# Ritesh622/Unbiased-Quantization-Distributed-Mean-Estimation

Hardware: AMD Instinct MI355X
Metric: quantize+dequantize M-vectors/sec at d=2^20 (1/2/4/8 GPU) + NMSE vs reference (higher is better)
Workload: dtype f32

## Files before the change

unbiased-quantization-distributed-mean-estimation_amd/csrc/uq_unbiased.hip:

```cpp
#include <hip/hip_runtime.h>

#include <algorithm>
#include <cstdint>
#include <type_traits>

#include "uq_internal.h"
#include "uq_unbiased_kernels.h"

namespace {

struct WsLayout {
    size_t agg_off, incl_off, map1_off, rec_off, cnt_off, part_off, l1_off, total;
    int32_t tiles;
    template <class T>
    T* at(void* ws, size_t off) const { return (T*)((char*)ws + off); }
    uint64_t* tile_row(void* ws, size_t off, int64_t j0) const { return at<uint64_t>(ws, off) + j0 * tiles; }
};

WsLayout layout(int64_t n, int64_t d, const L1Plan& plan) {
    WsLayout w{};
    const int64_t tiles = (d + kQTile - 1) / kQTile;
    w.tiles = (int32_t)tiles;
    w.agg_off = kCtrlBytes;
    w.incl_off = up256(w.agg_off + (size_t)n * tiles * sizeof(uint64_t));
// ... 72 lines not shown
    if (rc) return rc;
    if (n == 0) return UQ_OK;
    if (!l1_out) return fail(UQ_E_INVALID, "null l1_out");
    hipStream_t st = (hipStream_t)stream;
    if (d == 0) return hip_check(hipMemsetAsync(l1_out, 0, n * sizeof(float), st), "memset l1");
    return launch_l1(x, n, d, plan, w.at<float>(ws, w.part_off), l1_out, st);
}

}

namespace {

template <bool B>
using Flag = std::integral_constant<bool, B>;

template <class F>
bool select_qc(bool q, bool c, bool cv, F&& f) {
    constexpr Flag<true> Y{};
    constexpr Flag<false> N{};
    switch ((q ? 4 : 0) | (c ? 2 : 0) | (cv ? 1 : 0)) {
        case 5: f(Y, N, Y); return true;
        case 7: f(Y, Y, Y); return true;
        case 6: f(Y, Y, N); return true;
        case 3: f(N, Y, Y); return true;
        case 2: f(N, Y, N); return true;
        default: return false;
    }
}

template <class F>
bool select_vqc(bool v, bool q, bool c, bool cv, F&& f) {
    if (v) return select_qc(q, c, cv, [&](auto Q, auto C, auto CV) { f(Flag<true>{}, Q, C, CV); });
    return select_qc(q, c, cv, [&](auto Q, auto C, auto CV) { f(Flag<false>{}, Q, C, CV); });
}

int bad_selector() { return fail(UQ_E_INVALID, "internal: bad kernel selector"); }

struct PlanIn {
    int64_t n, d, ldo, ldc;
    bool x16, out16, codes16;
    bool has_out, has_codes, nib, l1_given;
    int slots;
};
struct ChunkPlan {
    int64_t nj;
    bool seg;
    int32_t prefixed, R, nseg;
};
struct UnbiasedPlan {
    int32_t form;
    bool V, Q, C, CV, l1_given;
    int64_t chunks;
    ChunkPlan last;
    int32_t tiles;
    size_t agg_off, map0_off, map1_off, rec_off, cnt_off;
};

int chunk_plan(const PlanIn& in, const UnbiasedPlan& p, int64_t j0, ChunkPlan* c) {
    c->nj = std::min<int64_t>(kMaxGridY, in.n - j0);
    const int64_t total_tiles = c->nj * (int64_t)p.tiles;
    c->seg = p.V && in.d <= ((int64_t)1 << 29) && total_tiles >= kSegMinTiles;
    c->R = 1;
    c->nseg = 1;
    if (c->seg) {
        int slots = in.slots;
        if (slots <= 0) {
            const int rc = stream_slots(&slots);
            if (rc) return rc;
        }
        const int64_t segs = std::max<int64_t>(1, slots / c->nj);
        c->R = (int32_t)((p.tiles + segs - 1) / segs);
        c->nseg = (p.tiles + c->R - 1) / c->R;
    }
    c->prefixed = c->nj >= 4 ? 1 : 0;
    return UQ_OK;
}

int plan_unbiased(const PlanIn& in, const WsLayout& w, UnbiasedPlan* p) {
    *p = UnbiasedPlan{};
    if (!in.has_out && !in.has_codes) return fail(UQ_E_INVALID, "nothing to write: out and codes are both NULL");
    const int64_t n = in.n, d = in.d;
    p->tiles = w.tiles;
    p->agg_off = w.agg_off;
    p->map0_off = w.incl_off;
    p->map1_off = w.map1_off;
    p->rec_off = w.rec_off;
    p->cnt_off = w.cnt_off;
    p->Q = in.has_out;
    p->C = in.has_codes;
    p->l1_given = in.l1_given;
    p->V = in.x16 && (!in.has_out || in.out16) && ((d % 4 == 0 && in.ldo % 4 == 0) || n == 1);
    p->CV = !in.has_codes || (in.codes16 && d % 16 == 0 && (in.ldc % 16 == 0 || n == 1));
    p->chunks = 1;
    p->last = ChunkPlan{n, false, 0, w.tiles, 1};
    if (!in.nib && d <= kSmallL1Max && p->V && n <= 0x7FFFFFFF) {
        p->form = UQ_FORM_SMALL;
        return UQ_OK;
    }
    const bool stream_form = n >= kStreamMinClients && p->V && d <= ((int64_t)1 << 29);
    if (in.nib) {
        if (!stream_form || !in.has_out || !in.has_codes)
            return fail(UQ_E_INVALID, "internal: 4-bit codes outside the stream form");
        p->form = UQ_FORM_STREAM_NIBBLES;
        p->CV = true;
        return UQ_OK;
    }
    if (stream_form) {
        p->form = UQ_FORM_STREAM;
        return UQ_OK;
    }
    p->chunks = (n + kMaxGridY - 1) / kMaxGridY;
    const int rc = chunk_plan(in, *p, (p->chunks - 1) * kMaxGridY, &p->last);
    if (rc) return rc;
    p->form = p->last.seg ? UQ_FORM_SEGMENTS : UQ_FORM_PHASED;
    return UQ_OK;
}

bool bad_pitches(bool has_out, int64_t ldo, bool has_codes, int64_t ldc, int64_t d, bool nib) {
    return (has_out && ldo < d) || (has_codes && ldc < (nib ? d / 2 : d));
}

bool bad_nibble_shape(int64_t n, int64_t d) {
    return n < kStreamMinClients || d % kNibAlign != 0 || d > ((int64_t)1 << 29);
}
int nibble_shape_error() {
    return fail(UQ_E_INVALID, "4-bit codes need n >= 256 and d a multiple of 4096 (<= 2^29)");
}

thread_local UnbiasedPlan t_last_plan{};

int export_plan(const UnbiasedPlan& p, int64_t* out, int32_t cap) {
    if (!out || cap < 0) return fail(UQ_E_INVALID, "null plan output");
    const int64_t f[UQ_PLAN_FIELDS] = {
        p.form, p.V, p.Q, p.C, p.CV, p.l1_given, p.chunks, p.last.nj, p.last.prefixed, p.last.R, p.last.nseg,
        p.tiles, (int64_t)p.agg_off, (int64_t)p.map0_off, (int64_t)p.map1_off, (int64_t)p.rec_off, (int64_t)p.cnt_off,
        (int64_t)sizeof(TileRec), kRecPerClient, kRecClients, kRecEvents, kFoldEvents};
    for (int i = 0; i < std::min<int32_t>(cap, UQ_PLAN_FIELDS); ++i) out[i] = f[i];
    return UQ_OK;
}

int unbiased_codes_impl(const float* x, float* out, int64_t ldo, int8_t* codes, int64_t ldc, int32_t* overflow,
                        int64_t n, int64_t d, int64_t m, const float* X, float Xval, const float* l1, float* l1_out,
                        int32_t T, void* ws, size_t ws_bytes, void* stream, bool nib = false) {
    L1Plan plan;
    WsLayout w;
    int rc = check_common(x, n, d, T, ws, ws_bytes, &plan, &w);
    if (rc) return rc;
    t_last_plan = UnbiasedPlan{};
    if (m < 0) return fail(UQ_E_INVALID, "m must be >= 0");
    if (bad_pitches(out, ldo, codes, ldc, d, nib)) return fail(UQ_E_INVALID, "row pitches must be >= d");
    if (n == 0 || d == 0) return UQ_OK;
    if (!X && n != 1) return fail(UQ_E_INVALID, "null X");
    const PlanIn in{n, d, ldo, ldc, aligned16(x), aligned16(out), aligned16(codes), out != nullptr, codes != nullptr,
                    nib, l1 != nullptr, 0};
    UnbiasedPlan P;
    rc = plan_unbiased(in, w, &P);
    if (rc) return rc;
    if (codes && !overflow) return fail(UQ_E_INVALID, "codes need a kmax[n] array");
    t_last_plan = P;
    hipStream_t st = (hipStream_t)stream;
    const float* l1use = l1;
    const float fm = (float)m;
    const bool vec4 = P.V, cvec = P.CV;
    if (P.form == UQ_FORM_SMALL) {
        if (!select_qc(out, codes, cvec, [&](auto Q, auto C, auto CV) {
                hipLaunchKernelGGL((quantize_small_kernel<Q(), C(), CV()>), dim3((unsigned)n), dim3(kQBlock), 0, st, x,
                                   out, codes, overflow, d, w.tiles, fm, X, Xval, l1, l1_out, ldo, ldc);
            }))
            return bad_selector();
        return hip_check(hipGetLastError(), "quantize_small_kernel launch");
    }
    if (!l1use) {
        float* l1buf = w.at<float>(ws, w.l1_off);
        rc = launch_l1(x, n, d, plan, w.at<float>(ws, w.part_off), l1buf, st);
        if (rc) return rc;
        l1use = l1buf;
    }
    if (l1_out && l1_out != l1use) {
        rc = hip_check(hipMemcpyAsync(l1_out, l1use, n * sizeof(float), hipMemcpyDeviceToDevice, st), "copy l1");
        if (rc) return rc;
    }
    const bool stream_form = P.form == UQ_FORM_STREAM || P.form == UQ_FORM_STREAM_NIBBLES;
    if (codes && !stream_form) {
        rc = hip_check(hipMemsetAsync(overflow, 0, n * sizeof(int32_t), st), "memset kmax");
        if (rc) return rc;
    }
    if (P.form == UQ_FORM_STREAM_NIBBLES) {
        hipLaunchKernelGGL((quantize_stream_kernel<true, true, true, true>), dim3((unsigned)n), dim3(kQBlock), 0, st, x,
                           out, codes, overflow, d, w.tiles, fm, X, Xval, l1use, w.tiles, 1, nullptr, ldo, ldc);
        return hip_check(hipGetLastError(), "quantize_stream_kernel (4-bit codes) launch");
    }
    if (P.form == UQ_FORM_STREAM) {
        if (!select_qc(out, codes, cvec, [&](auto Q, auto C, auto CV) {
                hipLaunchKernelGGL((quantize_stream_kernel<Q(), C(), CV()>), dim3((unsigned)n), dim3(kQBlock), 0, st, x,
                                   out, codes, overflow, d, w.tiles, fm, X, Xval, l1use, w.tiles, 1, nullptr, ldo, ldc);
            }))
            return bad_selector();
        return hip_check(hipGetLastError(), "quantize_stream_kernel launch");
    }
    for (int64_t j0 = 0; j0 < n; j0 += kMaxGridY) {
        ChunkPlan ck;
        rc = chunk_plan(in, P, j0, &ck);
        if (rc) return rc;
        const int64_t nj = ck.nj;
        const float* xj = x + j0 * d;
        float* outj = out ? out + j0 * ldo : nullptr;
        int8_t* codesj = codes ? codes + j0 * ldc : nullptr;
        int32_t* ovj = codes ? overflow + j0 : nullptr;
        const float* Xj = X ? X + j0 : nullptr;
        const float* l1j = l1use + j0;
        uint64_t* agg = w.tile_row(ws, w.agg_off, j0);
        uint64_t* pre = w.tile_row(ws, w.incl_off, j0);
        uint64_t* map1 = w.tile_row(ws, w.map1_off, j0);
        TileRec* recs = w.at<TileRec>(ws, w.rec_off);
        uint32_t* reccnt = w.at<uint32_t>(ws, w.cnt_off);
        const bool seg = ck.seg;
        const dim3 tgrid((unsigned)w.tiles, (unsigned)nj);
        const int32_t R = ck.R, nseg = ck.nseg;
        if (seg) {
            hipLaunchKernelGGL(agg_stream_kernel, dim3((unsigned)(nj * nseg)), dim3(kQBlock), 0, st, xj, d, w.tiles, fm,
                               l1j, R, nseg, agg, reccnt);
        } else if (vec4) {
            hipLaunchKernelGGL(tile_agg_kernel<true>, tgrid, dim3(kQBlock), 0, st, xj, d, w.tiles, fm, l1j, agg, reccnt);
        } else {
            hipLaunchKernelGGL(tile_agg_kernel<false>, tgrid, dim3(kQBlock), 0, st, xj, d, w.tiles, fm, l1j, agg, reccnt);
        }
        rc = hip_check(hipGetLastError(), "tile sums launch");
        if (rc) return rc;
        const int32_t prefixed = ck.prefixed;
        if (prefixed) {
            hipLaunchKernelGGL(tile_prefix_kernel, dim3((unsigned)nj), dim3(kQBlock), 0, st, agg, w.tiles);
            rc = hip_check(hipGetLastError(), "tile_prefix_kernel launch");
            if (rc) return rc;
        }
        const auto map_and_fold = [&](auto V) {
            hipLaunchKernelGGL((tile_map_kernel<V()>), tgrid, dim3(kQBlock), 0, st, xj, d, w.tiles, fm, l1j, agg, pre, map1,
                               recs, reccnt, prefixed);
            const int e = hip_check(hipGetLastError(), "tile_map_kernel launch");
            if (e) return e;
            hipLaunchKernelGGL((exact_fold_kernel<V()>), dim3((unsigned)nj), dim3(kQBlock), 0, st, xj, d, w.tiles, fm, l1j,
                               pre, map1, agg, recs, reccnt);
            return hip_check(hipGetLastError(), "exact_fold_kernel launch");
        };
        rc = vec4 ? map_and_fold(Flag<true>{}) : map_and_fold(Flag<false>{});
        if (rc) return rc;
        pre = agg;
        if (seg) {
            if (!select_qc(out, codes, cvec, [&](auto Q, auto C, auto CV) {
                    hipLaunchKernelGGL((quantize_stream_kernel<Q(), C(), CV()>), dim3((unsigned)(nj * nseg)),
                                       dim3(kQBlock), 0, st, xj, outj, codesj, ovj, d, w.tiles, fm, Xj, Xval, l1j, R, nseg,
                                       pre, ldo, ldc);
                }))
                return bad_selector();
            rc = hip_check(hipGetLastError(), "quantize_stream_kernel (segments) launch");
            if (rc) return rc;
            continue;
        }
        if (!select_vqc(vec4, out, codes, cvec, [&](auto V, auto Q, auto C, auto CV) {
                hipLaunchKernelGGL((tile_out_kernel<V(), Q(), C(), CV()>), tgrid, dim3(kQBlock), 0, st, xj, outj, codesj,
                                   ovj, d, w.tiles, fm, Xj, Xval, l1j, pre, ldo, ldc);
            }))
            return bad_selector();
        rc = hip_check(hipGetLastError(), "tile_out_kernel launch");
        if (rc) return rc;
    }
    return UQ_OK;
}

}

extern "C" {

int uq_type_unbiased_codes_ld_f32(const float* x, float* out, int64_t ldq, int8_t* codes, int64_t ldc,
                                  int32_t* overflow, int64_t n, int64_t d, int64_t m, const float* X, const float* l1,
                                  float* l1_out, int32_t T, void* ws, size_t ws_bytes, void* stream) {
    if (n > 0 && d > 0 && !X) return fail(UQ_E_INVALID, "null X");
    return unbiased_codes_impl(x, out, ldq, codes, ldc, overflow, n, d, m, X, 0.0f, l1, l1_out, T, ws, ws_bytes,
                               stream);
}

int uq_type_unbiased_nibbles_ld_f32(const float* x, float* out, int64_t ldq, uint8_t* nib, int64_t ldn,
                                    int32_t* kmax, int64_t n, int64_t d, int64_t m, const float* X, const float* l1,
                                    float* l1_out, int32_t T, void* ws, size_t ws_bytes, void* stream) {
    if (n < 0 || d < 0) return fail(UQ_E_INVALID, "n and d must be >= 0");
    if (n == 0 || d == 0) return UQ_OK;
    if (!x || !out || !nib || !kmax || !X) return fail(UQ_E_INVALID, "null pointer (x, out, codes, kmax and X are required)");
    if (bad_nibble_shape(n, d)) return nibble_shape_error();
    if (ldq < d || ldq % 4 != 0 || ldn < d / 2 || ldn % 16 != 0 || !aligned16(x) || !aligned16(out) || !aligned16(nib))
        return fail(UQ_E_INVALID, "4-bit codes need 16-byte aligned rows: ldq >= d, ldq % 4 == 0, ldn >= d/2, ldn % 16 == 0");
    return unbiased_codes_impl(x, out, ldq, (int8_t*)nib, ldn, kmax, n, d, m, X, 0.0f, l1, l1_out, T, ws, ws_bytes,
                               stream, true);
}

int uq_nibbles_q_mean_ld_f32(const uint8_t* nib, int64_t ldn, const float* q, int64_t ldq, const float* l1,
                             const int32_t* kmax, int64_t n, int64_t d, int64_t m, float n_div, int32_t accumulate,
                             float* est, void* stream) {
    if (n < 0 || d < 0 || m < 0) return fail(UQ_E_INVALID, "n, d and m must be >= 0");
    if (d == 0) return UQ_OK;
    if (!est || (n > 0 && (!nib || !l1 || !kmax || !q))) return fail(UQ_E_INVALID, "null pointer (q is required)");
    if (d % kNibAlign != 0 || ldq < d || ldq % 4 != 0 || ldn < d / 2 || ldn % 4 != 0 || !aligned16(est) ||
        (n > 0 && (!aligned16(q) || ((uintptr_t)nib & 3u))))
        return fail(UQ_E_INVALID, "4-bit code mean: d % 4096 == 0, ldq >= d (multiple of 4), ldn >= d/2 (multiple of 4), "
                                  "16-byte aligned est and q");
    const int64_t blocks = d / (kCodesMeanThreads * kMeanCpt);
    if (blocks > 0x7FFFFFFF) return fail(UQ_E_INVALID, "d too large");
    hipLaunchKernelGGL(nibbles_mean_kernel, dim3((unsigned)blocks), dim3(kCodesMeanThreads), 0, (hipStream_t)stream, nib,
                       ldn, l1, kmax, n, d, (float)m, n_div, accumulate, est, q, ldq);
    return hip_check(hipGetLastError(), "nibbles_mean_kernel launch");
}

int uq_type_unbiased_codes_f32(const float* x, float* out, int8_t* codes, int32_t* overflow, int64_t n, int64_t d,
                               int64_t m, const float* X, const float* l1, float* l1_out, int32_t T, void* ws,
                               size_t ws_bytes, void* stream) {
    return uq_type_unbiased_codes_ld_f32(x, out, d, codes, d, overflow, n, d, m, X, l1, l1_out, T, ws, ws_bytes,
                                         stream);
}

int uq_type_unbiased_vec_f32(const float* x, float* out, int64_t d, int64_t m, float X, int32_t T, void* ws,
                             size_t ws_bytes, void* stream) {
    if (d > 0 && !out) return fail(UQ_E_INVALID, "null out");
    return unbiased_codes_impl(x, out, d, nullptr, d, nullptr, 1, d, m, nullptr, X, nullptr, nullptr, T, ws, ws_bytes,
                               stream);
}

int uq_type_unbiased_f32(const float* x, float* out, int64_t n, int64_t d, int64_t m, const float* X,
                         const float* l1, float* l1_out, int32_t T, void* ws, size_t ws_bytes,
                         void* stream) {
    if (n > 0 && d > 0 && !out) return fail(UQ_E_INVALID, "null out");
    return uq_type_unbiased_codes_f32(x, out, nullptr, nullptr, n, d, m, X, l1, l1_out, T, ws, ws_bytes, stream);
}

int uq_codes_decode_f32(const int8_t* codes, const float* l1, int64_t n, int64_t d, int64_t m, float* out,
                        void* stream) {
    if (n < 0 || d < 0 || m < 0) return fail(UQ_E_INVALID, "n, d and m must be >= 0");
    if (n == 0 || d == 0) return UQ_OK;
    if (!codes || !l1 || !out) return fail(UQ_E_INVALID, "null pointer");
    hipStream_t st = (hipStream_t)stream;
    const int64_t chunks = (d + kDecChunk - 1) / kDecChunk;
    if (chunks > 0x7FFFFFFF) return fail(UQ_E_INVALID, "d too large");
    const bool vec = aligned16(codes) && aligned16(out) && d % 16 == 0;
    dim3 grid((unsigned)chunks, (unsigned)n);
    if (vec)
        hipLaunchKernelGGL(codes_decode_kernel<true>, grid, dim3(256), 0, st, codes, l1, d, (float)m, out);
    else
        hipLaunchKernelGGL(codes_decode_kernel<false>, grid, dim3(256), 0, st, codes, l1, d, (float)m, out);
    return hip_check(hipGetLastError(), "codes_decode_kernel launch");
}

int uq_codes_q_mean_ld_f32(const int8_t* codes, int64_t ldc, const float* q, int64_t ldq, const float* l1,
                           const int32_t* kmax, int64_t n, int64_t d, int64_t m, float n_div, int32_t accumulate,
                           float* est, void* stream) {
    if (n < 0 || d < 0 || m < 0) return fail(UQ_E_INVALID, "n, d and m must be >= 0");
    if (d == 0) return UQ_OK;
    if (!est || (n > 0 && (!codes || !l1 || !kmax))) return fail(UQ_E_INVALID, "null pointer");
    if (q && ldq < d) return fail(UQ_E_INVALID, "ldq must be >= d");
    if (ldc < d) return fail(UQ_E_INVALID, "ldc must be >= d");
    hipStream_t st = (hipStream_t)stream;
    const bool vec = (n == 0 || aligned16(codes)) && aligned16(est) && d % 16 == 0 && ldc % 16 == 0;
    const int64_t blocks = (d + kCodesMeanThreads * kMeanCpt - 1) / (kCodesMeanThreads * kMeanCpt);
    if (blocks > 0x7FFFFFFF) return fail(UQ_E_INVALID, "d too large");
    const dim3 tb(kCodesMeanThreads);
    if (vec && d % (kCodesMeanThreads * kMeanCpt) == 0)
        hipLaunchKernelGGL((codes_mean_kernel<true, true>), dim3((unsigned)blocks), tb, 0, st, codes, ldc, l1, kmax, n,
                           d, (float)m, n_div, accumulate, est, q, ldq);
    else if (vec)
        hipLaunchKernelGGL(codes_mean_kernel<true>, dim3((unsigned)blocks), tb, 0, st, codes, ldc, l1, kmax, n, d,
                           (float)m, n_div, accumulate, est, q, ldq);
    else
        hipLaunchKernelGGL(codes_mean_kernel<false>, dim3((unsigned)blocks), tb, 0, st, codes, ldc, l1, kmax, n, d,
                           (float)m, n_div, accumulate, est, q, ldq);
    return hip_check(hipGetLastError(), "codes_mean_kernel launch");
}

int uq_codes_q_mean_f32(const int8_t* codes, const float* q, int64_t ldq, const float* l1, const int32_t* kmax,
                        int64_t n, int64_t d, int64_t m, float n_div, int32_t accumulate, float* est, void* stream) {
    return uq_codes_q_mean_ld_f32(codes, d, q, ldq, l1, kmax, n, d, m, n_div, accumulate, est, stream);
}

int uq_codes_mean_f32(const int8_t* codes, const float* l1, const int32_t* kmax, int64_t n, int64_t d, int64_t m,
                      float n_div, int32_t accumulate, float* est, void* stream) {
    return uq_codes_q_mean_f32(codes, nullptr, d, l1, kmax, n, d, m, n_div, accumulate, est, stream);
}

int uq_client_mean_f32(const float* q, int64_t n, int64_t d, int64_t ld, float n_div, int32_t accumulate,
                       float* est, void* stream) {
    if (n < 0 || d < 0) return fail(UQ_E_INVALID, "n and d must be >= 0");
    if (ld < d) return fail(UQ_E_INVALID, "ld must be >= d");
    if (d == 0) return UQ_OK;
    if (!est || (n > 0 && !q)) return fail(UQ_E_INVALID, "null pointer");
    hipStream_t st = (hipStream_t)stream;
    const bool vec4 = (n == 0 || aligned16(q)) && aligned16(est) && (d % 4 == 0) && (ld % 4 == 0);
    const int64_t threads = (d + 3) / 4;
    dim3 grid((unsigned)((threads + kMeanThreads - 1) / kMeanThreads));
    if (vec4)
        hipLaunchKernelGGL(client_mean_kernel<true>, grid, dim3(kMeanThreads), 0, st, q, n, d, ld, n_div, accumulate, est);
    else
        hipLaunchKernelGGL(client_mean_kernel<false>, grid, dim3(kMeanThreads), 0, st, q, n, d, ld, n_div, accumulate, est);
    return hip_check(hipGetLastError(), "client_mean_kernel launch");
}

int uq_type_unbiased_mean_f32(const float* x, float* out, int64_t n, int64_t d, int64_t m, const float* X,
                              const float* l1, int32_t T, float n_div, int32_t accumulate, float* est,
                              void* ws, size_t ws_bytes, void* stream) {
    if (!out) return fail(UQ_E_INVALID, "out must be non-NULL in this version");
    int rc = uq_type_unbiased_f32(x, out, n, d, m, X, l1, nullptr, T, ws, ws_bytes, stream);
    if (rc) return rc;
    return uq_client_mean_f32(out, n, d, d, n_div, accumulate, est, stream);
}

int uq_test_unbiased_plan(int64_t n, int64_t d, int64_t ldq, int64_t ldc, int32_t x_aligned, int32_t out_aligned,
                          int32_t codes_aligned, int32_t has_out, int32_t has_codes, int32_t nib, int32_t l1_given,
                          int32_t slots, int64_t* plan_out, int32_t cap) {
    L1Plan l1plan;
    if (n < 0 || d < 0) return fail(UQ_E_INVALID, "n and d must be >= 0");
    if (n > (int64_t)1 << 31 || d > (int64_t)1 << 40) return fail(UQ_E_INVALID, "n or d too large");
    if (slots < 0) return fail(UQ_E_INVALID, "slots must be >= 0");
    if (!make_plan(d, 1, &l1plan)) return fail(UQ_E_INVALID, "cannot build L1 plan");
    const WsLayout w = layout(n, d, l1plan);
    if ((int64_t)w.tiles * n > 0xFFFFFFFFll) return fail(UQ_E_INVALID, "batch too large for one call");
    if (bad_pitches(has_out, ldq, has_codes, ldc, d, nib)) return fail(UQ_E_INVALID, "row pitches must be >= d");
    UnbiasedPlan P{};
    if (n > 0 && d > 0) {
        if (nib && bad_nibble_shape(n, d)) return nibble_shape_error();
        const PlanIn in{n, d, ldq, ldc, x_aligned != 0, out_aligned != 0, codes_aligned != 0, has_out != 0,
                        has_codes != 0, nib != 0, l1_given != 0, slots};
        const int rc = plan_unbiased(in, w, &P);
        if (rc) return rc;
    }
    return export_plan(P, plan_out, cap);
}

int uq_test_last_unbiased_plan(int64_t* plan_out, int32_t cap) { return export_plan(t_last_plan, plan_out, cap); }

}
```

unbiased-quantization-distributed-mean-estimation_amd/csrc/uq_unbiased_kernels.h:

```cpp

#ifndef UQ_UNBIASED_KERNELS_H
#define UQ_UNBIASED_KERNELS_H

#include "uq_common.h"

namespace {

constexpr int kQItems = 16;
constexpr int kQTile = kQBlock * kQItems;
constexpr int64_t kStreamMinClients = 256;
constexpr int64_t kSegMinTiles = 1024;

struct AbsOp {
    static constexpr bool kHist = false;
    float den, fm;
    uint32_t *h, *zn;
    __device__ static AbsOp make(const float*, float, int64_t) { return AbsOp{0.f, 0.f, nullptr, nullptr}; }
    __device__ float operator()(float v) const { return fabsf(v); }
    __device__ void apply4(const float (&v)[4], float (&a)[4]) const {
#pragma unroll
        for (int c = 0; c < 4; ++c) a[c] += fabsf(v[c]);
    }
};

// ... 1015 lines not shown
            if (tid == 0) {
                const TileRec* lr = reinterpret_cast<const TileRec*>(s_x);
                double S = P;
                for (uint32_t e = 0; e < lr->count; ++e) {
                    const EvEntry& ev = lr->ev[e];
                    S = S + ev.run;
                    if (ev.tie) {
                        S = S + (lowbit(S) ? ev.t1 : ev.t0);
                    } else {
                        for (int k = 0; k < kQItems; ++k) S = S + (double)ev.fr[k];
                    }
                }
                sl.misc[0] = S + lr->last_run;
            }
            __syncthreads();
            P = sl.misc[0];
            __syncthreads();
        } else {
            TileRegs r;
            load_tile<VEC4>(r, x, d, tiles, (uint32_t)idx, tid);
            stage_tile<VEC4>(r, s_x, tid);
            __syncthreads();
            const int64_t t0 = (int64_t)tile * kQTile;
            const int len = (int)((d - t0) < kQTile ? (d - t0) : kQTile);
            const Binade B = binade_of(P);
            TileState st;
            TileVals tv;
            if (len == kQTile)
                tile_pass1<true, true>(s_x, tv, sl, tid, len, dp, fm, B, st);
            else
                tile_pass1<false, true>(s_x, tv, sl, tid, len, dp, fm, B, st);
            double pnext;
            (void)resolve_exact(P, B, st, tv, s_x, sl, tid, pnext);
            __syncthreads();
            P = pnext;
        }
        Pb = (uint64_t)__double_as_longlong(P);
        ++tile;
    }
}

template <bool VEC4, bool WQ, bool WC, bool CVEC>
__global__ void __launch_bounds__(kQBlock)
tile_out_kernel(const float* __restrict__ x, float* __restrict__ out, int8_t* __restrict__ codes,
                int32_t* __restrict__ overflow, int64_t d, int32_t tiles, float fm, const float* __restrict__ Xs,
                float Xval, const float* __restrict__ l1, const uint64_t* __restrict__ pre, int64_t ldo, int64_t ldc) {
    __shared__ __attribute__((aligned(16))) float s_x[kQTile];
    __shared__ float s_tab[kTab];
    __shared__ ScanLds sl;
    const int tid = threadIdx.x;
    const int32_t tile = blockIdx.x;
    const int64_t vec = blockIdx.y;
    TileRegs r;
    load_tile<VEC4>(r, x, d, tiles, (uint32_t)(vec * tiles + tile), tid);
    const float L = l1[vec];
    build_table(s_tab, tid, L, fm);
    stage_tile<VEC4>(r, s_x, tid);
    __syncthreads();
    const int64_t t0 = (int64_t)tile * kQTile;
    const int len = (int)((d - t0) < kQTile ? (d - t0) : kQTile);
    const DivPlan dp = div_plan(L);
    const double P = __longlong_as_double((long long)pre[vec * tiles + tile]);
    const Binade B = binade_of(P);
    TileState st;
    TileVals tv;
    if (len == kQTile)
        tile_pass1<true, true>(s_x, tv, sl, tid, len, dp, fm, B, st);
    else
        tile_pass1<false, true>(s_x, tv, sl, tid, len, dp, fm, B, st);
    double pnext;
    const double base = resolve_exact(P, B, st, tv, s_x, sl, tid, pnext);
    uint32_t cw[4];
    float kmax = 0.0f;
    tile_pass2<WQ, WC>(s_x, tv, s_tab, tid, base, L, fm, Xs ? Xs[vec] : Xval, cw, kmax);
    if (WC) {
        store_codes<CVEC>(codes + vec * ldc + t0, cw, len, tid);
        publish_kmax(kmax, L, overflow, vec, tid);
    }
    __syncthreads();
    if (WQ) store_tile<VEC4>(s_x, out + vec * ldo + t0, len, tid);
}

constexpr int kMeanThreads = 1024;
template <bool VEC4>
__global__ void __launch_bounds__(kMeanThreads)
client_mean_kernel(const float* __restrict__ q, int64_t n, int64_t d, int64_t ld, float n_div, int accumulate,
                   float* __restrict__ est) {
    const int64_t col = ((int64_t)blockIdx.x * blockDim.x + threadIdx.x) * 4;
    if (col >= d) return;
    if (VEC4) {
        float4 e = accumulate ? *reinterpret_cast<const float4*>(est + col) : make_float4(0.f, 0.f, 0.f, 0.f);
        int64_t j = 0;
        for (; j + 8 <= n; j += 8) {
            float4 t[8];
#pragma unroll
            for (int u = 0; u < 8; ++u) t[u] = ld_stream(reinterpret_cast<const float4*>(q + (j + u) * ld + col));
#pragma unroll
            for (int u = 0; u < 8; ++u) {
                e.x += t[u].x / n_div; e.y += t[u].y / n_div;
                e.z += t[u].z / n_div; e.w += t[u].w / n_div;
            }
        }
        for (; j < n; ++j) {
            const float4 t = *reinterpret_cast<const float4*>(q + j * ld + col);
            e.x += t.x / n_div; e.y += t.y / n_div; e.z += t.z / n_div; e.w += t.w / n_div;
        }
        *reinterpret_cast<float4*>(est + col) = e;
    } else {
        const int cnt = (int)((d - col) < 4 ? (d - col) : 4);
        for (int k = 0; k < cnt; ++k) {
            float e = accumulate ? est[col + k] : 0.f;
            for (int64_t j = 0; j < n; ++j) e += q[j * ld + col + k] / n_div;
            est[col + k] = e;
        }
    }
}

constexpr int kDecChunk = 4096;
constexpr int kMeanClients = 32;

__device__ __forceinline__ float decode_one(int8_t c, const float* tab) {
    const int ci = (int)c;
    const int k = ci ^ (ci >> 31);
    return __uint_as_float(__float_as_uint(tab[k]) ^ ((uint32_t)ci & 0x80000000u));
}

template <bool VEC>
__global__ void __launch_bounds__(256)
codes_decode_kernel(const int8_t* __restrict__ codes, const float* __restrict__ l1, int64_t d, float fm,
                    float* __restrict__ out) {
    __shared__ float tab[128];
    const int64_t vec = blockIdx.y;
    const int tid = threadIdx.x;
    const float L = l1[vec];
    if (tid < 128) tab[tid] = (L * (float)tid) / fm;
    __syncthreads();
    const int64_t i0 = (int64_t)blockIdx.x * kDecChunk + (int64_t)tid * 16;
    const int8_t* cr = codes + vec * d;
    float* orow = out + vec * d;
    if (VEC && i0 + 16 <= d) {
        const uint4 w = *reinterpret_cast<const uint4*>(cr + i0);
        const uint32_t ws[4] = {w.x, w.y, w.z, w.w};
#pragma unroll
        for (int k4 = 0; k4 < 4; ++k4) {
            float o[4];
#pragma unroll
            for (int c = 0; c < 4; ++c) o[c] = decode_one((int8_t)((ws[k4] >> (8 * c)) & 0xFF), tab);
            *reinterpret_cast<float4*>(orow + i0 + 4 * k4) = make_float4(o[0], o[1], o[2], o[3]);
        }
    } else {
        for (int64_t i = i0; i < i0 + 16 && i < d; ++i) orow[i] = decode_one(cr[i], tab);
    }
}

constexpr int kMeanCpt = 8;
constexpr int kCodesMeanThreads = 512;
constexpr int kMeanUnroll = 16;
static_assert(kMeanClients == 2 * kMeanUnroll, "two code batches per table group");

__device__ __forceinline__ void mean_load_batch(uint2 (&w)[kMeanUnroll], const int8_t* cp, int64_t ldc) {
#pragma unroll
    for (int u = 0; u < kMeanUnroll; ++u) {
        const u32x2v t = __builtin_nontemporal_load(reinterpret_cast<const u32x2v*>(cp + (int64_t)u * ldc));
        w[u] = make_uint2(t.x, t.y);
    }
}

__device__ __forceinline__ void mean_add_batch(float (&e)[kMeanCpt], const uint2 (&w)[kMeanUnroll],
                                               const float (*tabn)[256], int jj) {
#pragma unroll
    for (int u = 0; u < kMeanUnroll; ++u) {
        const float* tb = tabn[jj + u];
#pragma unroll
        for (int k = 0; k < 4; ++k) e[k] += tb[(w[u].x >> (8 * k)) & 0xFF];
#pragma unroll
        for (int k = 0; k < 4; ++k) e[4 + k] += tb[(w[u].y >> (8 * k)) & 0xFF];
    }
}

__device__ __forceinline__ void mean_build_tables(float (*tabn)[256], const float* __restrict__ l1,
                                                  const int32_t* __restrict__ kmaxv, int64_t j0, int nb, int wid,
                                                  int lane, float fm, float n_div) {
    for (int jj = wid; jj < nb; jj += kCodesMeanThreads / kWave) {
        const float L = l1[j0 + jj];
        const int km = min(127, max(0, kmaxv[j0 + jj]));
        for (int k = lane; k <= km; k += kWave) {
            const float v = ((L * (float)k) / fm) / n_div;
            tabn[jj][k] = v;
            tabn[jj][255 - k] = -v;
        }
    }
}

__device__ __forceinline__ void mean_add_bytes(float (&e)[kMeanCpt], const int8_t* __restrict__ codes, int64_t ldc,
                                               const float (*tabn)[256], int64_t j0, int nb, int64_t i0, int64_t d) {
    for (int jj = 0; jj < nb; ++jj)
        for (int k = 0; k < kMeanCpt; ++k)
            if (i0 + k < d) e[k] += tabn[jj][(uint8_t)codes[(j0 + jj) * ldc + i0 + k]];
}

__device__ __forceinline__ uint32_t mean_ovf_mask(const int32_t* __restrict__ kmaxv, int64_t j0, int nb) {
    uint32_t mk = 0;
    for (int jj = 0; jj < nb; ++jj) mk |= (kmaxv[j0 + jj] > 127 ? 1u : 0u) << jj;
    return mk;
}

__device__ __forceinline__ void mean_add_mixed(float (&e)[kMeanCpt], const int8_t* __restrict__ codes, int64_t ldc,
                                            const float* __restrict__ q, int64_t ldq, const float (*tabn)[256],
                                            uint32_t ovf, int64_t j0, int nb, int64_t i0, int64_t d, float n_div) {
    for (int jj = 0; jj < nb; ++jj) {
        const int64_t j = j0 + jj;
        if ((ovf >> jj) & 1u) {
            for (int k = 0; k < kMeanCpt; ++k)
                if (i0 + k < d) e[k] += q[j * ldq + i0 + k] / n_div;
        } else {
            for (int k = 0; k < kMeanCpt; ++k)
                if (i0 + k < d) e[k] += tabn[jj][(uint8_t)codes[j * ldc + i0 + k]];
        }
    }
}

template <bool VEC, bool ALL = false>
__global__ void __launch_bounds__(kCodesMeanThreads)
codes_mean_kernel(const int8_t* __restrict__ codes, int64_t ldc, const float* __restrict__ l1,
                  const int32_t* __restrict__ kmaxv, int64_t n, int64_t d, float fm, float n_div, int accumulate,
                  float* __restrict__ est, const float* __restrict__ q, int64_t ldq) {
    __shared__ float tabn[kMeanClients][256];
    __shared__ uint32_t s_ovf;
    const int tid = threadIdx.x;
    const int lane = tid & (kWave - 1);
    const int wid = __builtin_amdgcn_readfirstlane(tid / kWave);
    const int64_t i0 = ((int64_t)blockIdx.x * kCodesMeanThreads + tid) * kMeanCpt;
    const bool full = ALL || (VEC && i0 + kMeanCpt <= d);
    float e[kMeanCpt];
#pragma unroll
    for (int k = 0; k < kMeanCpt; ++k) e[k] = (accumulate && i0 + k < d) ? est[i0 + k] : 0.0f;
    bool any = false;
    if (q) {
        if (tid == 0) s_ovf = 0u;
        __syncthreads();
        bool a = false;
        for (int64_t j = tid; j < n; j += kCodesMeanThreads) a = a || kmaxv[j] > 127;
        if (a) s_ovf = 1u;
        __syncthreads();
        any = s_ovf != 0u;
    }
    const int64_t groups = n / kMeanClients;
    if (any) {
        for (int64_t j0 = 0; j0 < n; j0 += kMeanClients) {
            const int nb = (int)min((int64_t)kMeanClients, n - j0);
            const uint32_t ovf = mean_ovf_mask(kmaxv, j0, nb);
            __syncthreads();
            mean_build_tables(tabn, l1, kmaxv, j0, nb, wid, lane, fm, n_div);
            __syncthreads();
            mean_add_mixed(e, codes, ldc, q, ldq, tabn, ovf, j0, nb, i0, d, n_div);
        }
    } else {
    const int8_t* cbase = codes + (full ? i0 : 0);
    uint2 wa[kMeanUnroll], wb[kMeanUnroll];
    if (VEC && groups > 0) mean_load_batch(wa, cbase, ldc);
    for (int64_t g = 0; g < groups; ++g) {
        const int64_t j0 = g * kMeanClients;
        __syncthreads();
        mean_build_tables(tabn, l1, kmaxv, j0, kMeanClients, wid, lane, fm, n_div);
        __syncthreads();
        if (VEC) {
            mean_load_batch(wb, cbase + (j0 + kMeanUnroll) * ldc, ldc);
            if (full) mean_add_batch(e, wa, tabn, 0);
            const int64_t jn = (j0 + kMeanClients + kMeanUnroll <= n) ? j0 + kMeanClients : n - kMeanUnroll;
            mean_load_batch(wa, cbase + jn * ldc, ldc);
            if (full) mean_add_batch(e, wb, tabn, kMeanUnroll);
        }
        if (!full) mean_add_bytes(e, codes, ldc, tabn, j0, kMeanClients, i0, d);
    }
    const int64_t jr = groups * kMeanClients;
    const int nr = (int)(n - jr);
    if (nr > 0) {
        __syncthreads();
        mean_build_tables(tabn, l1, kmaxv, jr, nr, wid, lane, fm, n_div);
        __syncthreads();
        if (full) {
            for (int jj = 0; jj < nr; ++jj) {
                const uint2 w = *reinterpret_cast<const uint2*>(codes + (jr + jj) * ldc + i0);
#pragma unroll
                for (int k = 0; k < 4; ++k) e[k] += tabn[jj][(w.x >> (8 * k)) & 0xFF];
#pragma unroll
                for (int k = 0; k < 4; ++k) e[4 + k] += tabn[jj][(w.y >> (8 * k)) & 0xFF];
            }
        } else {
            mean_add_bytes(e, codes, ldc, tabn, jr, nr, i0, d);
        }
    }
    }
    if (full) {
        *reinterpret_cast<float4*>(est + i0) = make_float4(e[0], e[1], e[2], e[3]);
        *reinterpret_cast<float4*>(est + i0 + 4) = make_float4(e[4], e[5], e[6], e[7]);
    } else {
        for (int k = 0; k < kMeanCpt; ++k)
            if (i0 + k < d) est[i0 + k] = e[k];
    }
}

constexpr int kNibMax = 7;
constexpr int64_t kNibAlign = kCodesMeanThreads * kMeanCpt;

__device__ __forceinline__ void nib_load_batch(uint32_t (&w)[kMeanUnroll], const uint8_t* cp, int64_t ldn) {
#pragma unroll
    for (int u = 0; u < kMeanUnroll; ++u) w[u] = __builtin_nontemporal_load(reinterpret_cast<const uint32_t*>(cp + (int64_t)u * ldn));
}

__device__ __forceinline__ void nib_add_batch(float (&e)[kMeanCpt], const uint32_t (&w)[kMeanUnroll],
                                              const float (*tab)[16], int jj) {
#pragma unroll
    for (int u = 0; u < kMeanUnroll; ++u) {
        const float* tb = tab[jj + u];
#pragma unroll
        for (int k = 0; k < kMeanCpt; ++k) e[k] += tb[(w[u] >> (4 * k)) & 0xFu];
    }
}

constexpr int kNibChunk = 1024;
__device__ __forceinline__ void nib_build_tables(float (*tab)[16], const float* __restrict__ l1,
                                                 const int32_t* __restrict__ kmaxv, int64_t j0, int nb, float fm,
                                                 float n_div) {
    for (int e = threadIdx.x; e < nb * 8; e += kCodesMeanThreads) {
        const int jj = e >> 3, k = e & 7;
        const float L = l1[j0 + jj];
        const int km = min(kNibMax, max(0, kmaxv[j0 + jj]));
        if (k <= km) {
            const float v = ((L * (float)k) / fm) / n_div;
            tab[jj][k] = v;
            tab[jj][15 - k] = -v;
        }
    }
}

__global__ void __launch_bounds__(kCodesMeanThreads)
nibbles_mean_kernel(const uint8_t* __restrict__ nib, int64_t ldn, const float* __restrict__ l1,
                    const int32_t* __restrict__ kmaxv, int64_t n, int64_t d, float fm, float n_div, int accumulate,
                    float* __restrict__ est, const float* __restrict__ q, int64_t ldq) {
    __shared__ float tab[kNibChunk][16];
    __shared__ uint32_t s_ovf;
    const int tid = threadIdx.x;
    const int64_t i0 = ((int64_t)blockIdx.x * kCodesMeanThreads + tid) * kMeanCpt;
    float e[kMeanCpt];
    if (accumulate) {
        const float4 a = *reinterpret_cast<const float4*>(est + i0), b = *reinterpret_cast<const float4*>(est + i0 + 4);
        e[0] = a.x; e[1] = a.y; e[2] = a.z; e[3] = a.w; e[4] = b.x; e[5] = b.y; e[6] = b.z; e[7] = b.w;
    } else {
#pragma unroll
        for (int k = 0; k < kMeanCpt; ++k) e[k] = 0.0f;
    }
    if (tid == 0) s_ovf = 0u;
    __syncthreads();
    bool a = false;
    for (int64_t j = tid; j < n; j += kCodesMeanThreads) a = a || kmaxv[j] > kNibMax;
    if (a) s_ovf = 1u;
    __syncthreads();
    const bool any = s_ovf != 0u;
    const uint8_t* cbase = nib + i0 / 2;
    for (int64_t c0 = 0; c0 < n; c0 += kNibChunk) {
        const int nc = (int)min((int64_t)kNibChunk, n - c0);
        __syncthreads();
        nib_build_tables(tab, l1, kmaxv, c0, nc, fm, n_div);
        __syncthreads();
        const int full = any ? 0 : nc / kMeanClients * kMeanClients;
        if (full > 0) {
            uint32_t wa[kMeanUnroll], wb[kMeanUnroll];
            const uint8_t* cb = cbase + c0 * ldn;
            nib_load_batch(wa, cb, ldn);
            for (int g = 0; g < full; g += kMeanClients) {
                nib_load_batch(wb, cb + (int64_t)(g + kMeanUnroll) * ldn, ldn);
                nib_add_batch(e, wa, tab, g);
                const int gn = (g + kMeanClients + kMeanUnroll <= nc) ? g + kMeanClients : nc - kMeanUnroll;
                nib_load_batch(wa, cb + (int64_t)gn * ldn, ldn);
                nib_add_batch(e, wb, tab, g + kMeanUnroll);
            }
        }
        for (int jj = full; jj < nc; ++jj) {
            const int64_t j = c0 + jj;
            if (kmaxv[j] > kNibMax) {
                const float4 a4 = *reinterpret_cast<const float4*>(q + j * ldq + i0);
                const float4 b4 = *reinterpret_cast<const float4*>(q + j * ldq + i0 + 4);
                const float qq[kMeanCpt] = {a4.x, a4.y, a4.z, a4.w, b4.x, b4.y, b4.z, b4.w};
#pragma unroll
                for (int k = 0; k < kMeanCpt; ++k) e[k] += qq[k] / n_div;
            } else {
                const uint32_t w = *reinterpret_cast<const uint32_t*>(cbase + j * ldn);
#pragma unroll
                for (int k = 0; k < kMeanCpt; ++k) e[k] += tab[jj][(w >> (4 * k)) & 0xFu];
            }
        }
    }
    *reinterpret_cast<float4*>(est + i0) = make_float4(e[0], e[1], e[2], e[3]);
    *reinterpret_cast<float4*>(est + i0 + 4) = make_float4(e[4], e[5], e[6], e[7]);
}

}

#endif
```

Baseline: 0.4180.

## Restructure 4-bit code mean kernel with buffer loads, ring prefetch, and per-chunk overflow

Rewrites the nibble mean kernel to use 1024 threads with 4 codes per thread, so each thread loads one 16-bit value per client row through raw buffer loads. Out-of-range rows get a zero-size resource, which removes explicit bounds branches. Loads are prefetched in a two-stage ring of 16-row batches, and the LUT gathers are software-pipelined with byte-offset arithmetic and sched barriers. The old whole-array overflow pre-scan is replaced by overflow detection folded into per-chunk table building. The aim is more memory-level parallelism and less per-element index math, at the cost of more registers and narrower loads per thread.

```diff
diff --git a/unbiased-quantization-distributed-mean-estimation_amd/csrc/uq_unbiased.hip b/unbiased-quantization-distributed-mean-estimation_amd/csrc/uq_unbiased.hip
--- a/unbiased-quantization-distributed-mean-estimation_amd/csrc/uq_unbiased.hip
+++ b/unbiased-quantization-distributed-mean-estimation_amd/csrc/uq_unbiased.hip
@@ -398,9 +398,9 @@
         (n > 0 && (!aligned16(q) || ((uintptr_t)nib & 3u))))
         return fail(UQ_E_INVALID, "4-bit code mean: d % 4096 == 0, ldq >= d (multiple of 4), ldn >= d/2 (multiple of 4), "
                                   "16-byte aligned est and q");
-    const int64_t blocks = d / (kCodesMeanThreads * kMeanCpt);
+    const int64_t blocks = d / kNibAlign;
     if (blocks > 0x7FFFFFFF) return fail(UQ_E_INVALID, "d too large");
-    hipLaunchKernelGGL(nibbles_mean_kernel, dim3((unsigned)blocks), dim3(kCodesMeanThreads), 0, (hipStream_t)stream, nib,
+    hipLaunchKernelGGL(nibbles_mean_kernel, dim3((unsigned)blocks), dim3(kNibThreads), 0, (hipStream_t)stream, nib,
                        ldn, l1, kmax, n, d, (float)m, n_div, accumulate, est, q, ldq);
     return hip_check(hipGetLastError(), "nibbles_mean_kernel launch");
 }
diff --git a/unbiased-quantization-distributed-mean-estimation_amd/csrc/uq_unbiased_kernels.h b/unbiased-quantization-distributed-mean-estimation_amd/csrc/uq_unbiased_kernels.h
--- a/unbiased-quantization-distributed-mean-estimation_amd/csrc/uq_unbiased_kernels.h
+++ b/unbiased-quantization-distributed-mean-estimation_amd/csrc/uq_unbiased_kernels.h
@@ -1341,98 +1341,151 @@
 }
 
 constexpr int kNibMax = 7;
-constexpr int64_t kNibAlign = kCodesMeanThreads * kMeanCpt;
-
-__device__ __forceinline__ void nib_load_batch(uint32_t (&w)[kMeanUnroll], const uint8_t* cp, int64_t ldn) {
-#pragma unroll
-    for (int u = 0; u < kMeanUnroll; ++u) w[u] = __builtin_nontemporal_load(reinterpret_cast<const uint32_t*>(cp + (int64_t)u * ldn));
-}
-
-__device__ __forceinline__ void nib_add_batch(float (&e)[kMeanCpt], const uint32_t (&w)[kMeanUnroll],
-                                              const float (*tab)[16], int jj) {
-#pragma unroll
-    for (int u = 0; u < kMeanUnroll; ++u) {
-        const float* tb = tab[jj + u];
-#pragma unroll
-        for (int k = 0; k < kMeanCpt; ++k) e[k] += tb[(w[u] >> (4 * k)) & 0xFu];
+constexpr int kNibThreads = 1024;
+constexpr int kNibCpt = 4;
+constexpr int64_t kNibAlign = kNibThreads * kNibCpt;
+
+constexpr int kNibBatch = 16;
+constexpr int kNibRing = 2;
+constexpr uint32_t kNibRowBytes = kNibThreads * kNibCpt / 2;
+
+__device__ __forceinline__ void nib_load_batch(uint16_t (&w)[kNibBatch], const uint8_t* rows, int64_t ldn, int jj,
+                                               int nc, uint32_t voff) {
+    const uint8_t* row = rows + (int64_t)jj * ldn;
+#pragma unroll
+    for (int u = 0; u < kNibBatch; ++u, row += ldn)
+        w[u] = __builtin_amdgcn_raw_buffer_load_b16(make_rsrc(row, jj + u < nc ? kNibRowBytes : 0u), voff, 0,
+                                                              kAuxNT);
+}
+
+constexpr int kNibSub = 4;
+typedef uint16_t u16x2v __attribute__((ext_vector_type(2)));
+__device__ __forceinline__ void nib_gather(float (&v)[kNibSub][kNibCpt], const uint16_t (&w)[kNibBatch],
+                                           const char* tb, uint32_t row0, int u0) {
+#pragma unroll
+    for (int s = 0; s < kNibSub; s += 2) {
+        const u16x2v pr = {w[u0 + s], w[u0 + s + 1]};
+        const uint32_t m = __builtin_bit_cast(uint32_t, pr);
+        uint32_t lo = (m << 2) & 0x3C3C3C3Cu, hi = (m >> 2) & 0x3C3C3C3Cu;
+        asm("" : "+v"(lo), "+v"(hi));
+#pragma unroll
+        for (int k = 0; k < 2 * kNibCpt; ++k) {
+            const uint32_t off = (((k & 1) ? hi : lo) >> (8 * (k >> 1))) & 0xFFu;
+            v[s + k / kNibCpt][k % kNibCpt] =
+                *reinterpret_cast<const float*>(tb + (row0 + off) + (u0 + s + k / kNibCpt) * 64);
+        }
+    }
+}
+
+template <bool TAIL>
+__device__ __forceinline__ void nib_add_batch(float (&e)[kNibCpt], const uint16_t (&w)[kNibBatch],
+                                              const float (*tab)[16], uint32_t jj, int cnt) {
+    static_assert(sizeof(tab[0]) == 64 && kNibSub % 2 == 0 && kNibBatch % kNibSub == 0, "table row: 16 floats");
+    const uint32_t row0 = jj * 64u;
+    const char* tb = reinterpret_cast<const char*>(tab);
+    if (TAIL) {
+#pragma unroll
+        for (int u = 0; u < kNibBatch; ++u) {
+            if (u >= cnt) continue;
+#pragma unroll
+            for (int k = 0; k < kNibCpt; ++k) e[k] += tab[jj + u][((uint32_t)w[u] >> (4 * k)) & 0xFu];
+        }
+        return;
+    }
+    float v[2][kNibSub][kNibCpt];
+    nib_gather(v[0], w, tb, row0, 0);
+#pragma unroll
+    for (int g = 0; g < kNibBatch / kNibSub; ++g) {
+        if (g + 1 < kNibBatch / kNibSub) nib_gather(v[(g + 1) & 1], w, tb, row0, (g + 1) * kNibSub);
+        __builtin_amdgcn_sched_barrier(0);
+#pragma unroll
+        for (int s = 0; s < kNibSub; ++s)
+#pragma unroll
+            for (int k = 0; k < kNibCpt; ++k) e[k] += v[g & 1][s][k];
+        __builtin_amdgcn_sched_barrier(0);
     }
 }
 
 constexpr int kNibChunk = 1024;
-__device__ __forceinline__ void nib_build_tables(float (*tab)[16], const float* __restrict__ l1,
+__device__ __forceinline__ bool nib_build_tables(float (*tab)[16], const float* __restrict__ l1,
                                                  const int32_t* __restrict__ kmaxv, int64_t j0, int nb, float fm,
                                                  float n_div) {
-    for (int e = threadIdx.x; e < nb * 8; e += kCodesMeanThreads) {
+    bool ovf = false;
+    for (int e = threadIdx.x; e < nb * 8; e += kNibThreads) {
         const int jj = e >> 3, k = e & 7;
         const float L = l1[j0 + jj];
-        const int km = min(kNibMax, max(0, kmaxv[j0 + jj]));
+        const int kmj = kmaxv[j0 + jj];
+        ovf = ovf || kmj > kNibMax;
+        const int km = min(kNibMax, max(0, kmj));
         if (k <= km) {
             const float v = ((L * (float)k) / fm) / n_div;
             tab[jj][k] = v;
             tab[jj][15 - k] = -v;
         }
     }
-}
-
-__global__ void __launch_bounds__(kCodesMeanThreads)
+    return ovf;
+}
+
+__global__ void __launch_bounds__(kNibThreads)
 nibbles_mean_kernel(const uint8_t* __restrict__ nib, int64_t ldn, const float* __restrict__ l1,
                     const int32_t* __restrict__ kmaxv, int64_t n, int64_t d, float fm, float n_div, int accumulate,
                     float* __restrict__ est, const float* __restrict__ q, int64_t ldq) {
     __shared__ float tab[kNibChunk][16];
-    __shared__ uint32_t s_ovf;
+    __shared__ uint32_t s_ovf[2];
     const int tid = threadIdx.x;
-    const int64_t i0 = ((int64_t)blockIdx.x * kCodesMeanThreads + tid) * kMeanCpt;
-    float e[kMeanCpt];
+    const int64_t i0 = ((int64_t)blockIdx.x * kNibThreads + tid) * kNibCpt;
+    float e[kNibCpt];
     if (accumulate) {
-        const float4 a = *reinterpret_cast<const float4*>(est + i0), b = *reinterpret_cast<const float4*>(est + i0 + 4);
-        e[0] = a.x; e[1] = a.y; e[2] = a.z; e[3] = a.w; e[4] = b.x; e[5] = b.y; e[6] = b.z; e[7] = b.w;
+        const float4 a = *reinterpret_cast<const float4*>(est + i0);
+        e[0] = a.x; e[1] = a.y; e[2] = a.z; e[3] = a.w;
     } else {
 #pragma unroll
-        for (int k = 0; k < kMeanCpt; ++k) e[k] = 0.0f;
-    }
-    if (tid == 0) s_ovf = 0u;
-    __syncthreads();
-    bool a = false;
-    for (int64_t j = tid; j < n; j += kCodesMeanThreads) a = a || kmaxv[j] > kNibMax;
-    if (a) s_ovf = 1u;
-    __syncthreads();
-    const bool any = s_ovf != 0u;
+        for (int k = 0; k < kNibCpt; ++k) e[k] = 0.0f;
+    }
+    if (tid < 2) s_ovf[tid] = 0u;
+    const uint8_t* rows = nib + (int64_t)blockIdx.x * kNibRowBytes;
+    const uint32_t voff = (uint32_t)tid * (kNibCpt / 2);
     const uint8_t* cbase = nib + i0 / 2;
-    for (int64_t c0 = 0; c0 < n; c0 += kNibChunk) {
-        const int nc = (int)min((int64_t)kNibChunk, n - c0);
-        __syncthreads();
-        nib_build_tables(tab, l1, kmaxv, c0, nc, fm, n_div);
-        __syncthreads();
-        const int full = any ? 0 : nc / kMeanClients * kMeanClients;
-        if (full > 0) {
-            uint32_t wa[kMeanUnroll], wb[kMeanUnroll];
-            const uint8_t* cb = cbase + c0 * ldn;
-            nib_load_batch(wa, cb, ldn);
-            for (int g = 0; g < full; g += kMeanClients) {
-                nib_load_batch(wb, cb + (int64_t)(g + kMeanUnroll) * ldn, ldn);
-                nib_add_batch(e, wa, tab, g);
-                const int gn = (g + kMeanClients + kMeanUnroll <= nc) ? g + kMeanClients : nc - kMeanUnroll;
-                nib_load_batch(wa, cb + (int64_t)gn * ldn, ldn);
-                nib_add_batch(e, wb, tab, g + kMeanUnroll);
+    int par = 0;
+    for (int64_t c0 = 0; c0 < n; c0 += kNibChunk, par ^= 1) {
+        const int nc = __builtin_amdgcn_readfirstlane((int)min((int64_t)kNibChunk, n - c0));
+        __syncthreads();
+        if (nib_build_tables(tab, l1, kmaxv, c0, nc, fm, n_div)) s_ovf[par] = 1u;
+        if (tid == 0) s_ovf[par ^ 1] = 0u;
+        __syncthreads();
+        const int fast = __builtin_amdgcn_readfirstlane(s_ovf[par] != 0u ? 0 : nc);
+        if (fast > 0) {
+            uint16_t w[kNibRing][kNibBatch];
+            const uint8_t* crow = rows + c0 * ldn;
+#pragma unroll
+            for (int r = 0; r < kNibRing - 1; ++r) nib_load_batch(w[r], crow, ldn, r * kNibBatch, fast, voff);
+            for (int g0 = 0; g0 < fast; g0 += kNibRing * kNibBatch) {
+#pragma unroll
+                for (int r = 0; r < kNibRing; ++r) {
+                    const int g = g0 + r * kNibBatch;
+                    nib_load_batch(w[(r + kNibRing - 1) % kNibRing], crow, ldn, g + (kNibRing - 1) * kNibBatch, fast, voff);
+                    if (g + kNibBatch <= fast)
+                        nib_add_batch<false>(e, w[r], tab, (uint32_t)g, kNibBatch);
+                    else if (g < fast)
+                        nib_add_batch<true>(e, w[r], tab, (uint32_t)g, fast - g);
+                }
             }
         }
-        for (int jj = full; jj < nc; ++jj) {
+        for (int jj = fast; jj < nc; ++jj) {
             const int64_t j = c0 + jj;
             if (kmaxv[j] > kNibMax) {
                 const float4 a4 = *reinterpret_cast<const float4*>(q + j * ldq + i0);
-                const float4 b4 = *reinterpret_cast<const float4*>(q + j * ldq + i0 + 4);
-                const float qq[kMeanCpt] = {a4.x, a4.y, a4.z, a4.w, b4.x, b4.y, b4.z, b4.w};
-#pragma unroll
-                for (int k = 0; k < kMeanCpt; ++k) e[k] += qq[k] / n_div;
+                const float qq[kNibCpt] = {a4.x, a4.y, a4.z, a4.w};
+#pragma unroll
+                for (int k = 0; k < kNibCpt; ++k) e[k] += qq[k] / n_div;
             } else {
-                const uint32_t w = *reinterpret_cast<const uint32_t*>(cbase + j * ldn);
-#pragma unroll
-                for (int k = 0; k < kMeanCpt; ++k) e[k] += tab[jj][(w >> (4 * k)) & 0xFu];
+                const uint32_t w = *reinterpret_cast<const uint16_t*>(cbase + j * ldn);
+#pragma unroll
+                for (int k = 0; k < kNibCpt; ++k) e[k] += tab[jj][(w >> (4 * k)) & 0xFu];
             }
         }
     }
     *reinterpret_cast<float4*>(est + i0) = make_float4(e[0], e[1], e[2], e[3]);
-    *reinterpret_cast<float4*>(est + i0 + 4) = make_float4(e[4], e[5], e[6], e[7]);
 }
 
 }
```

After: 0.4040. 0.966x the previous value.
